# qic999/PCTrans

Measured on AMD Instinct MI355X. Metric: MSDeformAttn+decoder fwd samples/sec at 512x512, 100 queries, higher is better.
Workload: dtype bf16 decoder (autocast) / f32 MSDeformAttn pixel decoder

## Files before the change

include/pctrans_hip.h:

```cpp
#ifndef PCTRANS_HIP_H_
#define PCTRANS_HIP_H_

#include <stdint.h>

#ifdef __cplusplus
extern "C" {
#endif

#define PCT_ABI_VERSION 1

#define PCT_API __attribute__((visibility("default")))

#define PCT_OK 0
#define PCT_ERR_BAD_ARG (-1)
#define PCT_ERR_IM2COL_STEP (-2)
#define PCT_ERR_ALIGNMENT (-3)
#define PCT_ERR_UNSUPPORTED (-4)

PCT_API int pct_abi_version(void);
PCT_API const char *pct_error_string(int code);
PCT_API const char *pct_build_info(void);
PCT_API int pct_prepare_device(void);

PCT_API int pct_ms_deform_attn_forward_f32(const float *value, const int64_t *spatial_shapes, const int64_t *level_start,
// ... 7 lines not shown
PCT_API int pct_ms_deform_attn_forward_f16(const void *value, const int64_t *spatial_shapes, const int64_t *level_start,
                                   const float *sampling_loc, const float *attn_weight, int batch,
                                   int spatial_size, int num_heads, int channels, int num_levels, int num_query,
                                   int num_point, int im2col_step, void *output, void *stream);
PCT_API int pct_ms_deform_attn_forward_bf16(const void *value, const int64_t *spatial_shapes, const int64_t *level_start,
                                    const float *sampling_loc, const float *attn_weight, int batch,
                                    int spatial_size, int num_heads, int channels, int num_levels, int num_query,
                                    int num_point, int im2col_step, void *output, void *stream);

PCT_API int pct_ms_deform_attn_fused_forward_f32(const float *value, const int64_t *spatial_shapes,
                                                 const int64_t *level_start, const float *ref_points,
                                                 long long ref_batch_stride, const float *offsets,
                                                 const float *attn_logits, int batch, int spatial_size, int num_heads,
                                                 int channels, int num_levels, int num_query, int num_point,
                                                 float *output, void *stream);

PCT_API int pct_ms_deform_attn_forward_planes_f32(const float *value_planes, const int64_t *spatial_shapes,
                                                  const int64_t *level_start, const float *loc_planes,
                                                  const float *attn_planes, const float *ref_points,
                                                  long long ref_batch_stride, int batch, int spatial_size, int num_heads,
                                                  int channels, int num_levels, int num_query, int num_point,
                                                  float *output, void *stream);

PCT_API int pct_ms_deform_attn_backward_f32(const float *value, const int64_t *spatial_shapes, const int64_t *level_start,
                                    const float *sampling_loc, const float *attn_weight, const float *grad_output,
                                    int batch, int spatial_size, int num_heads, int channels, int num_levels,
                                    int num_query, int num_point, int im2col_step, float *grad_value,
                                    float *grad_sampling_loc, float *grad_attn_weight, void *stream);
PCT_API int pct_ms_deform_attn_backward_f64(const double *value, const int64_t *spatial_shapes, const int64_t *level_start,
                                    const double *sampling_loc, const double *attn_weight,
                                    const double *grad_output, int batch, int spatial_size, int num_heads,
                                    int channels, int num_levels, int num_query, int num_point, int im2col_step,
                                    double *grad_value, double *grad_sampling_loc, double *grad_attn_weight,
                                    void *stream);

PCT_API int pct_dynamic_mask_head_forward(const float *mask_feat, const float *ref_points, const float *params,
                                          int batch, int channels, int num_query, int height, int width, int stride,
                                          int rel_coord, int target_h, int target_w, int out_dtype, void *up_logits,
                                          unsigned char *attn_mask, void *stream);

PCT_API int pct_dynamic_mask_head_forward_mfma(const float *mask_feat, const float *ref_points, const float *params,
                                               int batch, int channels, int num_query, int height, int width,
                                               int stride, int rel_coord, int target_h, int target_w, void *scratch,
                                               void *up_logits, unsigned char *attn_mask, void *stream);

PCT_API int pct_dynamic_mask_head_forward_fused_bf16(const float *mask_feat, const float *ref_points, const float *params,
                                                     int batch, int channels, int num_query, int height, int width,
                                                     int stride, int rel_coord, int target_h, int target_w,
                                                     void *workspace, void *up_logits, unsigned char *attn_mask,
                                                     void *stream);

#include "pctrans_hip_train.h"
#include "pctrans_hip_post.h"

PCT_API int pct_add_layernorm_f32(const float *x, const float *y, const float *gamma, const float *beta, float eps,
                                  long long rows, int cols, float *out, void *stream);

PCT_API int pct_groupnorm_flatten_f32(const float *x, const float *gamma, const float *beta, int batch, int channels,
                                      int hw, int groups, float eps, float *stats, float *out,
                                      long long out_batch_stride, long long out_offset, void *stream);

PCT_API int pct_linear_k128_f32(const float *x, long long ldx, const float *x_add, long long ld_add, long long add_period,
                                const float *w, const float *bias, long long rows, int n, int act, float *y,
                                long long ldy, void *stream);
PCT_API void pct_msda_set_kernel_choice(int choice);
PCT_API int pct_msda_last_kernel(void);
PCT_API void pct_msda_set_bwd_kernel_choice(int choice);
PCT_API int pct_msda_last_bwd_kernel(void);

PCT_API int pct_linear_k128_multi_f32(const float *x, long long ldx, const float *x_add, long long ld_add,
                                      long long add_period, int nseg, const float *const *w, const float *const *bias,
                                      const int *n, const int *use_add, float *const *y, const long long *ldy,
                                      long long rows, void *stream);
PCT_API int pct_linear_k128_add_layernorm_f32(const float *x, long long ldx, const float *w, const float *bias,
                                              const float *residual, long long ldr, const float *gamma,
                                              const float *beta, float eps, long long rows, float *out,
                                              long long ldo, void *stream);

PCT_API int pct_linear_add_layernorm_f32(const float *x, long long ldx, int k, const float *w, void *w_split_ws,
                                         const float *bias, const float *residual, long long ldr, const float *gamma,
                                         const float *beta, float eps, long long rows, float *out, long long ldo,
                                         void *stream);

PCT_API int pct_ffn_layernorm_f32(const float *x, long long ldx, const float *w1, const float *b1, const float *w2,
                                  const float *b2, const float *gamma, const float *beta, float eps, int hidden,
                                  long long rows, void *w_image_ws, float *out, long long ldo, void *stream);

PCT_API int pct_conv1x1_groupnorm_tokens_f32(const float *x, const float *w, const float *bias, void *w_split_ws,
                                             const float *gamma, const float *beta, int groups, float eps, int batch,
                                             int in_channels, int out_channels, int hw, float *partial_ws, float *stats,
                                             float *out, long long out_batch_stride, long long out_offset, void *stream);

PCT_API int pct_conv1x1_nchw_f32(const float *x, const float *w, const float *bias, void *w_split_ws, int batch,
                                 int in_channels, int out_channels, int hw, float *out, void *stream);

PCT_API int pct_lsap_f32(const float *cost, int batch, int num_query, int ld_target, const int *num_target,
                         int *row_for_target, int *status, void *stream);

PCT_API int pct_masked_attention_bf16(const void *q, const void *k, const void *vT, const unsigned char *mask,
                                      int batch, int heads, int num_query, int num_key, int head_dim,
                                      int v_head_dim, float scale, int out_dtype, void *out, void *stream);

PCT_API int pct_cross_attention_bf16(const void *q_content, const void *q_pos, const void *k_content, const void *k_pos,
                                     const void *v, const unsigned char *mask, const unsigned char *row_open, int batch,
                                     int heads, int num_query, int num_key, float scale, void *out, void *stream);

// ... 5 lines not shown
```

pctrans_amd/_lib.py:

```python
import ctypes
import os

_HERE = os.path.dirname(os.path.abspath(__file__))
LIB_PATH = os.path.join(_HERE, "lib", "libpctrans_hip.so")
ABI_VERSION = 1

_lib = None

_vp, _i = ctypes.c_void_p, ctypes.c_int
_FWD_ARGS = [_vp, _vp, _vp, _vp, _vp, _i, _i, _i, _i, _i, _i, _i, _i, _vp, _vp]
_BWD_ARGS = [_vp, _vp, _vp, _vp, _vp, _vp, _i, _i, _i, _i, _i, _i, _i, _i, _vp, _vp, _vp, _vp]

SYMBOLS = {
    "pct_abi_version": ([], _i),
    "pct_error_string": ([_i], ctypes.c_char_p),
    "pct_build_info": ([], ctypes.c_char_p),
    "pct_prepare_device": ([], _i),
    "pct_ms_deform_attn_forward_f32": (_FWD_ARGS, _i),
    "pct_ms_deform_attn_forward_f64": (_FWD_ARGS, _i),
    "pct_ms_deform_attn_forward_f16": (_FWD_ARGS, _i),
    "pct_ms_deform_attn_forward_bf16": (_FWD_ARGS, _i),
    "pct_ms_deform_attn_backward_f32": (_BWD_ARGS, _i),
    "pct_ms_deform_attn_backward_f64": (_BWD_ARGS, _i),
    "pct_ms_deform_attn_fused_forward_f32": ([_vp, _vp, _vp, _vp, ctypes.c_longlong, _vp, _vp] + [_i] * 7 + [_vp, _vp], _i),
# ... 4 lines not shown
    "pct_msda_set_kernel_choice": ([_i], None),
    "pct_msda_last_kernel": ([], _i),
    "pct_msda_set_bwd_kernel_choice": ([_i], None),
    "pct_msda_last_bwd_kernel": ([], _i),
    "pct_linear_k128_multi_f32": ([_vp, ctypes.c_longlong, _vp, ctypes.c_longlong, ctypes.c_longlong, _i, _vp, _vp, _vp, _vp,
                                   _vp, _vp, ctypes.c_longlong, _vp], _i),
    "pct_linear_k128_add_layernorm_f32": ([_vp, ctypes.c_longlong, _vp, _vp, _vp, ctypes.c_longlong, _vp, _vp,
                                           ctypes.c_float, ctypes.c_longlong, _vp, ctypes.c_longlong, _vp], _i),
    "pct_linear_add_layernorm_f32": ([_vp, ctypes.c_longlong, _i, _vp, _vp, _vp, _vp, ctypes.c_longlong, _vp, _vp,
                                      ctypes.c_float, ctypes.c_longlong, _vp, ctypes.c_longlong, _vp], _i),
    "pct_groupnorm_flatten_f32": ([_vp, _vp, _vp, _i, _i, _i, _i, ctypes.c_float, _vp, _vp, ctypes.c_longlong,
                                   ctypes.c_longlong, _vp], _i),
    "pct_conv1x1_nchw_f32": ([_vp, _vp, _vp, _vp, _i, _i, _i, _i, _vp, _vp], _i),
    "pct_conv1x1_groupnorm_tokens_f32": ([_vp] * 6 + [_i, ctypes.c_float] + [_i] * 4 + [_vp, _vp, _vp, ctypes.c_longlong,
                                          ctypes.c_longlong, _vp], _i),
    "pct_ffn_layernorm_f32": ([_vp, ctypes.c_longlong, _vp, _vp, _vp, _vp, _vp, _vp, ctypes.c_float, _i, ctypes.c_longlong, _vp, _vp,
                               ctypes.c_longlong, _vp], _i),
    "pct_lsap_f32": ([_vp, _i, _i, _i, _vp, _vp, _vp, _vp], _i),
    "pct_cross_attention_bf16": ([_vp] * 7 + [_i] * 4 + [ctypes.c_float, _vp, _vp], _i),
    "pct_masked_attention_bf16": ([_vp, _vp, _vp, _vp] + [_i] * 6 + [ctypes.c_float, _i, _vp, _vp], _i),
    "pct_dynamic_mask_head_forward_mfma": ([_vp, _vp, _vp] + [_i] * 9 + [_vp, _vp, _vp, _vp], _i),
    "pct_dynamic_mask_head_forward_fused_bf16": ([_vp, _vp, _vp] + [_i] * 9 + [_vp, _vp, _vp, _vp], _i),
    "pct_dynamic_mask_head_forward": ([_vp, _vp, _vp] + [_i] * 10 + [_vp, _vp, _vp], _i),
}

OPT_IN_SYMBOLS = {
    "pct_dynamic_mask_head_backward_f32": ([_vp, _vp, _vp, _vp] + [_i] * 7 + [_vp, _vp, _vp, _vp, _vp], _i,
                                           "tests/test_dmh_train_gpu.py"),
    "pct_point_sample_f32": ([_vp, _vp, _vp] + [_i] * 7 + [_vp, _vp], _i, "tests/test_point_loss_gpu.py"),
    "pct_point_mask_loss_forward_f32": ([_vp, _vp, _i, _i, _i, _vp, _vp, _i, _i, _i, _vp, _i, _i, _vp, _vp, _vp, _vp], _i,
                                        "tests/test_point_loss_gpu.py"),
    "pct_point_mask_loss_backward_f32": ([_vp] * 6 + [_i] * 4 + [_vp, _vp], _i, "tests/test_point_loss_gpu.py"),
    "pct_point_select_uncertain_f32": ([_vp, _vp, _i, _i, _i, _vp, _i, _i, _i, _vp, _i, _vp, _vp], _i,
                                       "tests/test_point_select_gpu.py"),
    "pct_point_match_cost_f32": ([_vp, _i, _i, _i, _i, _vp, _i, _i, _i, _vp, _vp, _i, _vp, _i, ctypes.c_float, ctypes.c_float,
                                  _vp, _vp, _vp], _i, "tests/test_match_cost_gpu.py"),
    "pct_instance_label_map_f32": ([_vp, _i, _i, _i, _vp, _vp, _i, _i, _i, _vp, _vp], _i, "tests/test_embedding_loss_gpu.py"),
    "pct_discriminative_loss_forward_f32": ([_vp, _vp] + [_i] * 5 + [ctypes.c_float] * 5 + [_vp] * 5, _i,
                                            "tests/test_embedding_loss_gpu.py"),
    "pct_discriminative_loss_backward_f32": ([_vp] * 4 + [_i] * 5 + [ctypes.c_float, _vp, _vp], _i,
                                             "tests/test_embedding_loss_gpu.py"),
}

_POST_MASKS = [_vp] + [_i] * 7 + [_vp, _vp, _vp]
_POST_LABELS = [_vp] + [_i] * 7 + [_vp, _vp, _vp]
POST_SYMBOLS = {
    "pct_instance_masks_f32": (_POST_MASKS, _i, "tests/test_postprocess_gpu.py"),
    "pct_instance_masks_bf16": (_POST_MASKS, _i, "tests/test_postprocess_gpu.py"),
    "pct_instance_labels_from_bits": ([_vp, _vp] + [_i] * 5 + [_vp, _vp, _vp], _i, "tests/test_postprocess_gpu.py"),
    "pct_instance_labels_f32": (_POST_LABELS, _i, "tests/test_postprocess_gpu.py"),
    "pct_instance_labels_bf16": (_POST_LABELS, _i, "tests/test_postprocess_gpu.py"),
}


class PctransLibraryError(RuntimeError):
    pass


def lib():
    global _lib
    if _lib is not None:
        return _lib
    if not os.path.exists(LIB_PATH):
        raise PctransLibraryError(
            "libpctrans_hip.so not found at %s -- build it with `make -C pctrans_amd/csrc` "
            "(or `python -c 'import __graft_entry__ as g; g.build()'`).  "
            "pctrans_amd has no CPU / eager fallback for device tensors." % LIB_PATH)
    l = ctypes.CDLL(LIB_PATH)
    for name, (argtypes, restype) in list(SYMBOLS.items()) + [
            (k, v[:2]) for k, v in list(OPT_IN_SYMBOLS.items()) + list(POST_SYMBOLS.items())]:
        try:
            fn = getattr(l, name)
        except AttributeError as e:
            raise PctransLibraryError("libpctrans_hip.so does not export %s (stale build?)" % name) from e
        fn.argtypes = argtypes
        fn.restype = restype
    v = l.pct_abi_version()
    if v != ABI_VERSION:
        raise PctransLibraryError("libpctrans_hip.so ABI version %d, expected %d -- rebuild" % (v, ABI_VERSION))
    _lib = l
    return _lib


def check(code, what):
    if code != 0:
        msg = lib().pct_error_string(code).decode()
        raise RuntimeError("%s failed: %s (code %d)" % (what, msg, code))


_PREPARED = set()


def prepare_device(device):
    import torch
    idx = device.index if device.index is not None else torch.cuda.current_device()
    if idx in _PREPARED:
        return
    if torch.cuda.is_current_stream_capturing():
        return
    with torch.cuda.device(idx):
        check(lib().pct_prepare_device(), "prepare_device")
    _PREPARED.add(idx)
```

pctrans_amd/csrc/c_abi.hip:

```cpp
#include <hip/hip_runtime.h>
#include <stdint.h>

#include "launchers.hpp"
#include "msda_common.hpp"

namespace {

int check_common(const void *value, const int64_t *shapes, const int64_t *starts, const void *loc,
                 const void *attn, int N, int S, int M, int D, int L, int Lq, int P, int im2col_step,
                 size_t elem, size_t loc_elem)
{
  if (N < 0 || S < 0 || Lq < 0 || M <= 0 || D <= 0 || L <= 0 || P <= 0 || im2col_step <= 0) return PCT_ERR_BAD_ARG;
  if (N == 0) return PCT_OK;
  const int step = N < im2col_step ? N : im2col_step;
  if (N % step != 0) return PCT_ERR_IM2COL_STEP;
  if (Lq == 0) return PCT_OK;
  if (!value || !shapes || !starts || !loc || !attn) return PCT_ERR_BAD_ARG;
  if ((long long)S * M * D >= 0x7fffffffLL) return PCT_ERR_UNSUPPORTED;
  if ((uintptr_t)value % elem || (uintptr_t)loc % loc_elem || (uintptr_t)attn % loc_elem ||
      (uintptr_t)shapes % 8 || (uintptr_t)starts % 8)
    return PCT_ERR_ALIGNMENT;
  return PCT_OK;
}

// ... 96 lines not shown
}

int instance_labels_impl(const void *logits, int bf16, int batch, int num_query, int h, int w, int height, int width, int dataset,
                         void *workspace, int16_t *labels, void *stream)
{
  const int rc = check_instance_post(batch, num_query, h, w, height, width, dataset);
  if (rc != PCT_OK || batch == 0) return rc;
  if (num_query == 0) return instance_labels_empty(batch, height, width, labels, stream);
  if (!logits || !workspace || !labels) return PCT_ERR_BAD_ARG;
  if (((uintptr_t)logits & (bf16 ? 1u : 3u)) || ((uintptr_t)workspace & 15u) || ((uintptr_t)labels & 1u)) return PCT_ERR_ALIGNMENT;
  return pct::launch_instance_labels(logits, bf16, batch, num_query, h, w, height, width, dataset, workspace, labels,
                                     static_cast<hipStream_t>(stream));
}

}

extern "C" {

int pct_instance_masks_f32(const float *logits, int batch, int num_query, int h, int w, int height, int width, int dataset,
                           uint32_t *bits, int32_t *areas, void *stream)
{
  return instance_masks_impl(logits, 0, batch, num_query, h, w, height, width, dataset, bits, areas, stream);
}

int pct_instance_masks_bf16(const void *logits, int batch, int num_query, int h, int w, int height, int width, int dataset,
                            uint32_t *bits, int32_t *areas, void *stream)
{
  return instance_masks_impl(logits, 1, batch, num_query, h, w, height, width, dataset, bits, areas, stream);
}

int pct_instance_labels_from_bits(const uint32_t *bits, const int32_t *areas, int batch, int num_query, int height, int width,
                                  int dataset, void *workspace, int16_t *labels, void *stream)
{
  const int rc = check_instance_post(batch, num_query, 1, 1, height, width, dataset);
  if (rc != PCT_OK || batch == 0) return rc;
  if (num_query == 0) return instance_labels_empty(batch, height, width, labels, stream);
  if (!bits || !areas || !workspace || !labels) return PCT_ERR_BAD_ARG;
  if (((uintptr_t)bits & 15u) || ((uintptr_t)areas & 3u) || ((uintptr_t)workspace & 15u) || ((uintptr_t)labels & 1u))
    return PCT_ERR_ALIGNMENT;
  return pct::launch_instance_labels_from_bits(bits, areas, batch, num_query, height, width, dataset, workspace, labels,
                                               static_cast<hipStream_t>(stream));
}

int pct_instance_labels_f32(const float *logits, int batch, int num_query, int h, int w, int height, int width, int dataset,
                            void *workspace, int16_t *labels, void *stream)
{
  return instance_labels_impl(logits, 0, batch, num_query, h, w, height, width, dataset, workspace, labels, stream);
}

int pct_instance_labels_bf16(const void *logits, int batch, int num_query, int h, int w, int height, int width, int dataset,
                             void *workspace, int16_t *labels, void *stream)
{
  return instance_labels_impl(logits, 1, batch, num_query, h, w, height, width, dataset, workspace, labels, stream);
}

int pct_abi_version(void) { return PCT_ABI_VERSION; }

const char *pct_error_string(int code)
{
  switch (code) {
    case PCT_OK: return "ok";
    case PCT_ERR_BAD_ARG: return "bad argument (null pointer or non-positive size)";
    case PCT_ERR_IM2COL_STEP: return "batch must be divisible by min(batch, im2col_step)";
    case PCT_ERR_ALIGNMENT: return "pointer not aligned to its element size";
    case PCT_ERR_UNSUPPORTED: return "shape not supported by the gfx950 kernels";
    default: break;
  }
  if (code > 0) return hipGetErrorString(static_cast<hipError_t>(code));
  return "unknown error";
}

int pct_ms_deform_attn_forward_f32(const float *value, const int64_t *spatial_shapes, const int64_t *level_start,
                                   const float *sampling_loc, const float *attn_weight, int batch,
                                   int spatial_size, int num_heads, int channels, int num_levels, int num_query,
                                   int num_point, int im2col_step, float *output, void *stream)
{
  return forward_impl<float, float>(value, spatial_shapes, level_start, sampling_loc, attn_weight, batch,
                                    spatial_size, num_heads, channels, num_levels, num_query, num_point,
                                    im2col_step, output, stream);
}

int pct_ms_deform_attn_forward_f64(const double *value, const int64_t *spatial_shapes, const int64_t *level_start,
                                   const double *sampling_loc, const double *attn_weight, int batch,
                                   int spatial_size, int num_heads, int channels, int num_levels, int num_query,
                                   int num_point, int im2col_step, double *output, void *stream)
{
  return forward_impl<double, double>(value, spatial_shapes, level_start, sampling_loc, attn_weight, batch,
                                      spatial_size, num_heads, channels, num_levels, num_query, num_point,
                                      im2col_step, output, stream);
}

int pct_ms_deform_attn_forward_f16(const void *value, const int64_t *spatial_shapes, const int64_t *level_start,
                                   const float *sampling_loc, const float *attn_weight, int batch,
                                   int spatial_size, int num_heads, int channels, int num_levels, int num_query,
                                   int num_point, int im2col_step, void *output, void *stream)
{
  return forward_impl<pct::half_bits, float>(value, spatial_shapes, level_start, sampling_loc, attn_weight, batch,
                                             spatial_size, num_heads, channels, num_levels, num_query, num_point,
                                             im2col_step, output, stream);
}

int pct_ms_deform_attn_forward_bf16(const void *value, const int64_t *spatial_shapes, const int64_t *level_start,
                                    const float *sampling_loc, const float *attn_weight, int batch,
                                    int spatial_size, int num_heads, int channels, int num_levels, int num_query,
                                    int num_point, int im2col_step, void *output, void *stream)
{
// ... 435 lines not shown
```

pctrans_amd/csrc/launchers.hpp:

```cpp
#pragma once
#include <hip/hip_runtime.h>
#include <stdint.h>

#include "../../include/pctrans_hip.h"

namespace pct {

constexpr int PCT_NOT_COVERED = -100;

enum MsdaFwdKernel { MSDA_FWD_AUTO = 0, MSDA_FWD_WIN = 1, MSDA_FWD_GENERIC = 2, MSDA_FWD_QUAD = 3, MSDA_FWD_COL = 4 };
enum MsdaBwdKernel { MSDA_BWD_AUTO = 0, MSDA_BWD_WIN = 1, MSDA_BWD_GENERIC = 2, MSDA_BWD_COL = 3 };

template <typename T>
int launch_msda_forward(const void *value, const int64_t *shapes, const int64_t *starts, const void *loc, const void *attn, int N,
                        int S, int M, int D, int L, int Lq, int P, void *out, hipStream_t stream);
template <typename T>
int launch_msda_forward_special(const void *value, const int64_t *shapes, const int64_t *starts, const void *loc,
                                const void *attn, int N, int S, int M, int D, int L, int Lq, int P, void *out, hipStream_t stream,
                                const float *ref, long long ref_batch_stride);
int launch_msda_forward_planes(const void *value, const int64_t *shapes, const int64_t *starts, const void *loc, const void *attn,
                               int N, int S, int M, int D, int L, int Lq, int P, void *out, hipStream_t stream, const float *ref,
                               long long ref_batch_stride);
template <typename T>
int launch_msda_forward_win(const void *value, const int64_t *shapes, const int64_t *starts, const void *loc, const void *attn,
// ... 22 lines not shown
int launch_msda_backward_win(const float *value, const int64_t *shapes, const int64_t *starts, const float *loc,
                             const float *attn, const float *grad_out, int N, int S, int M, int D, int L, int Lq, int P,
                             float *grad_value, float *grad_loc, float *grad_attn, hipStream_t stream);
int launch_msda_backward_col(const float *value, const int64_t *shapes, const int64_t *starts, const float *loc,
                             const float *attn, const float *grad_out, int N, int S, int M, int D, int L, int Lq, int P,
                             float *grad_value, float *grad_loc, float *grad_attn, bool forced, hipStream_t stream);
void set_msda_bwd_kernel_choice(int c);
int msda_bwd_kernel_choice();
void note_msda_bwd_kernel(int k);
int msda_bwd_last_kernel();

unsigned *win_queue_slot(hipStream_t stream);
int prepare_win_queue_device();
int prepare_msda_backward_col_device();
int prepare_ffn_device();

int launch_dyn_mask_head(const float *feat, const float *ref, const float *params, int N, int C, int Q, int H, int W, int stride,
                         int rel_coord, int th, int tw, int out_dtype, void *up, unsigned char *amask, hipStream_t stream);
int launch_dyn_mask_head_mfma(const float *feat, const float *ref, const float *params, int N, int C, int Q, int H, int W,
                              int stride, int rel_coord, int th, int tw, void *scratch, void *up, unsigned char *amask,
                              hipStream_t stream);
int launch_dyn_mask_head_fused(const float *feat, const float *ref, const float *params, int N, int C, int Q, int H, int W,
                               int stride, int rel_coord, int th, int tw, void *workspace, void *up, unsigned char *amask,
                               hipStream_t stream);
int launch_dyn_mask_head_bwd(const float *feat, const float *ref, const float *params, const float *grad_up, int N, int C, int Q,
                             int H, int W, int stride, int rel_coord, void *workspace, float *grad_feat, float *grad_ref,
                             float *grad_params, hipStream_t stream);

int launch_linear_k128(const float *x, long long ldx, const float *x2, long long ldx2, long long x2_period, const float *w,
                       const float *bias, long long rows, int n, int epi, float *y, long long ldy, const float *residual,
                       long long ldr, const float *gamma, const float *beta, float eps, hipStream_t stream);
int launch_linear_k128_split(const float *x, long long ldx, const float *x2, long long ldx2, long long x2_period, const float *w,
                             const float *bias, long long rows, int n, int epi, float *y, long long ldy, const float *residual,
                             long long ldr, const float *gamma, const float *beta, float eps, hipStream_t stream);
int launch_linear_k128_split_multi(const float *x, long long ldx, const float *x2, long long ldx2, long long x2_period, int nseg,
                                   const float *const *w, const float *const *bias, const int *n, const int *use_add,
                                   float *const *y, const long long *ldy, long long rows, hipStream_t stream);
int launch_linear_ln_split(const float *x, long long ldx, const float *w, unsigned short *w_pieces, int K, const float *bias,
                           const float *residual, long long ldr, const float *gamma, const float *beta, float eps, long long rows,
                           float *out, long long ldo, hipStream_t stream);
int launch_ffn_fused_split(const float *x, long long ldx, const float *w1, const float *b1, const float *w2, const float *b2,
                           const float *gamma, const float *beta, float eps, int F, long long rows, void *img_ws, float *out,
                           long long ldo, hipStream_t stream);
int launch_conv1x1_nchw_split(const float *x, const float *w, const float *bias, unsigned short *w_split_ws, int N, int K, int HW,
                              float *y, hipStream_t stream);
int launch_conv1x1_groupnorm_tokens(const float *x, const float *w, const float *bias, unsigned short *w_split_ws,
                                    const float *gamma, const float *beta, float eps, int N, int K, int HW, float *partial_ws,
                                    float *stats, float *out, long long out_batch_stride, hipStream_t stream);
int launch_add_layernorm(const float *x, const float *y, const float *gamma, const float *beta, float eps, long long rows,
                         int cols, float *out, hipStream_t stream);
int launch_groupnorm_flatten(const float *x, const float *gamma, const float *beta, int N, int C, int HW, int groups, float eps,
                             float *stats, float *out, long long out_batch_stride, long long out_offset, hipStream_t stream);

int launch_masked_attention(const void *q, const void *k, const void *vT, const unsigned char *mask, int N, int heads, int Q,
                            int S, int head_dim, int v_head_dim, float scale, int out_dtype, void *out, hipStream_t stream);
int launch_cross_attention(const void *q_c, const void *q_s, const void *k_c, const void *k_p, const void *v,
                           const unsigned char *mask, const unsigned char *row_open, int N, int heads, int Q, int S, float scale,
                           void *out, hipStream_t stream);
int launch_lsap(const float *cost, int batch, int num_query, int ld_target, const int *num_target, int *row_for_target,
                int *status, hipStream_t stream);

int launch_point_sample(const float *planes, const int *plane_index, const float *coords, int num_planes, int H, int W, int K,
                        int P, int per_row, float *out, hipStream_t stream);
int launch_point_loss_forward(const float *pred, const int *src_index, int num_pred, int H, int W, const float *tgt,
                              const int *tgt_index, int num_tgt, int Ht, int Wt, const float *coords, int K, int P, float *x,
                              float *t, float *sums, hipStream_t stream);
int launch_point_loss_backward(const float *x, const float *t, const float *coords, const float *alpha, const float *beta,
                               const float *gamma, int K, int P, int H, int W, float *grad_planes, hipStream_t stream);
int launch_point_select(const float *pred, const int *src_index, int num_pred, int H, int W, const float *cand_coords, int K, int S,
                        int num_keep, float *out_coords, int out_row_points, int *out_index, hipStream_t stream);
int launch_point_match_cost(const float *pred, int B, int Q, int H, int W, const float *tgt, int num_tgt, int Ht, int Wt,
                            const int *tgt_start, const int *tgt_count, int Gmax, const float *coords, int P, float cost_mask,
                            float cost_dice, void *workspace, float *cost, hipStream_t stream);

int launch_instance_label_map(const float *planes, int num_planes, int Ht, int Wt, const int *start, const int *count, int B, int h,
                              int w, int *labels, hipStream_t stream);
int launch_emb_loss_forward(const float *emb, const int *labels, int B, int E, int h, int w, int L, float delta_v, float delta_d,
                            float alpha, float beta, float gama, void *workspace, float *table, float *loss, int *status,
                            hipStream_t stream);
int launch_emb_loss_backward(const float *emb, const int *labels, const float *table, const float *grad_out, int B, int E, int h,
                             int w, int L, float delta_v, float *grad_emb, hipStream_t stream);

int instance_geometry_status(int N, int Q, int H, int W);
int launch_instance_masks(const void *logits, int bf16, int N, int Q, int h, int w, int H, int W, int dataset, unsigned *bits,
                          int *areas, hipStream_t stream);
int launch_instance_labels_from_bits(const unsigned *bits, const int *areas, int N, int Q, int H, int W, int dataset,
                                     void *workspace, short *labels, hipStream_t stream);
int launch_instance_labels(const void *logits, int bf16, int N, int Q, int h, int w, int H, int W, int dataset, void *workspace,
                           short *labels, hipStream_t stream);

}
```

pctrans_amd/fused_ops.py:

```python
import contextlib

import torch
from torch.nn import functional as F

from . import _lib, _timing


def _fusable(*tensors):
    if torch.is_grad_enabled() and any(t is not None and t.requires_grad for t in tensors):
        return False
    return all(t is None or (t.is_cuda and t.dtype == torch.float32) for t in tensors)


def add_layer_norm(x, y, norm):
    cols = x.shape[-1]
    if (not _fusable(x, y, norm.weight, norm.bias) or cols not in (64, 128, 256) or norm.weight is None
            or norm.bias is None or tuple(norm.normalized_shape) != (cols,) or (y is not None and y.shape != x.shape)):
        return norm(x if y is None else x + y)
    xc = x.contiguous()
    yc = y.contiguous() if y is not None else None
    out = torch.empty_like(xc)
    rows = xc.numel() // cols
    with torch.cuda.device(x.device):
        rc = _lib.lib().pct_add_layernorm_f32(
# ... 235 lines not shown
            and w.dtype == torch.float32 and w.device == x.device and tuple(w.shape[2:]) == (1, 1) and w.shape[0] == 128
            and w.shape[1] == x.shape[1] and w.shape[1] % 16 == 0 and (x.shape[2] * x.shape[3]) % 128 == 0
            and tuple(conv.stride) == (1, 1) and tuple(conv.padding) == (0, 0) and tuple(conv.dilation) == (1, 1)
            and conv.groups == 1 and getattr(conv, "norm", None) is None and getattr(conv, "activation", None) is None
            and x.numel() > 0 and x.shape[0] * (x.shape[2] * x.shape[3] // 128) < 2 ** 31 - 1
            and x.data_ptr() % 16 == 0 and w.data_ptr() % 16 == 0 and w.is_contiguous()
            and (conv.bias is None or conv.bias.data_ptr() % 16 == 0) and not torch.is_autocast_enabled()
            and not (torch.is_grad_enabled() and (x.requires_grad or w.requires_grad)))


def conv1x1_nchw(x, conv):
    if not conv1x1_nchw_supported(x, conv):
        return conv(x)
    n, k, h, w_ = x.shape
    stream = torch.cuda.current_stream(x.device).cuda_stream
    key = (x.device, stream, k)
    ws = _CONV_WS.get(key)
    if ws is None:
        ws = _CONV_WS[key] = torch.empty((3, 128, k), dtype=torch.bfloat16, device=x.device)
    out = torch.empty((n, 128, h, w_), dtype=torch.float32, device=x.device)
    with torch.cuda.device(x.device), _timing.timed("conv1x1 k=%d" % k, x):
        rc = _lib.lib().pct_conv1x1_nchw_f32(
            x.data_ptr(), conv.weight.data_ptr(), conv.bias.data_ptr() if conv.bias is not None else None, ws.data_ptr(),
            n, k, 128, h * w_, out.data_ptr(), stream)
    _lib.check(rc, "conv1x1_nchw")
    return out


def conv1x1_groupnorm_tokens_supported(x, conv, gn):
    return (conv1x1_nchw_supported(x, conv) and isinstance(gn, torch.nn.GroupNorm) and gn.num_groups == 32
            and gn.num_channels == 128 and gn.weight is not None and gn.bias is not None
            and gn.weight.data_ptr() % 16 == 0 and gn.bias.data_ptr() % 16 == 0 and x.shape[0] <= 65535
            and not (torch.is_grad_enabled() and gn.weight.requires_grad))


def conv1x1_groupnorm_tokens_into(x, conv, gn, out, row_offset):
    n, k, h, w_ = x.shape
    hw = h * w_
    stream = torch.cuda.current_stream(x.device).cuda_stream
    key = (x.device, stream, k)
    ws = _CONV_WS.get(key)
    if ws is None:
        ws = _CONV_WS[key] = torch.empty((3, 128, k), dtype=torch.bfloat16, device=x.device)
    partial = torch.empty((n * (hw // 128) * 2 * 64,), dtype=torch.float32, device=x.device)
    stats = torch.empty((n * 64,), dtype=torch.float32, device=x.device)
    with torch.cuda.device(x.device), _timing.timed("conv1x1_gn k=%d" % k, x):
        rc = _lib.lib().pct_conv1x1_groupnorm_tokens_f32(
            x.data_ptr(), conv.weight.data_ptr(), conv.bias.data_ptr() if conv.bias is not None else None, ws.data_ptr(),
            gn.weight.data_ptr(), gn.bias.data_ptr(), 32, float(gn.eps), n, k, 128, hw, partial.data_ptr(), stats.data_ptr(),
            out.data_ptr(), out.stride(0), row_offset * 128, stream)
    _lib.check(rc, "conv1x1_groupnorm_tokens")


def groupnorm_flatten_supported(x, gn):
    return (x.is_cuda and x.dtype == torch.float32 and x.dim() == 4 and x.shape[1] == 128 and x.is_contiguous()
            and isinstance(gn, torch.nn.GroupNorm) and gn.num_channels == 128 and (128 // gn.num_groups) % 4 == 0
            and gn.weight is not None and gn.bias is not None and not torch.is_autocast_enabled()
            and not (torch.is_grad_enabled() and (x.requires_grad or gn.weight.requires_grad)))


def groupnorm_flatten_into(x, gn, out, row_offset):
    n, c, h, w = x.shape
    stats = torch.empty((n * gn.num_groups * 2,), dtype=torch.float32, device=x.device)
    with torch.cuda.device(x.device):
        rc = _lib.lib().pct_groupnorm_flatten_f32(
            x.data_ptr(), gn.weight.data_ptr(), gn.bias.data_ptr(), n, c, h * w, gn.num_groups, float(gn.eps),
            stats.data_ptr(), out.data_ptr(), out.stride(0), row_offset * c,
            torch.cuda.current_stream(x.device).cuda_stream)
    _lib.check(rc, "groupnorm_flatten")


def lsap_supported(cost):
    return cost.is_cuda and cost.dim() == 3 and cost.shape[1] <= 1024 and cost.shape[2] <= 512


def lsap(cost, num_target):
    c = cost.detach().float().contiguous()
    B, Q, Gm = c.shape
    nt = num_target.to(device=c.device, dtype=torch.int32).contiguous()
    rows = torch.empty((B, Gm), dtype=torch.int32, device=c.device)
    status = torch.empty((B,), dtype=torch.int32, device=c.device)
    with torch.cuda.device(c.device):
        rc = _lib.lib().pct_lsap_f32(c.data_ptr(), B, Q, Gm, nt.data_ptr(), rows.data_ptr(), status.data_ptr(),
                                     torch.cuda.current_stream(c.device).cuda_stream)
    _lib.check(rc, "lsap")
    return rows, status


def masked_attention_supported(q, k, v, num_heads, attn_mask, key_padding_mask, dropout_p, training, need_weights):
    if not (q.is_cuda and q.dtype == torch.bfloat16 and k.dtype == torch.bfloat16 and v.dtype == torch.bfloat16):
        return False
    if torch.is_grad_enabled() and (q.requires_grad or k.requires_grad or v.requires_grad):
        return False
    if need_weights or key_padding_mask is not None or (dropout_p > 0.0 and training):
        return False
    if q.shape[2] // num_heads not in (16, 32) or v.shape[2] // num_heads != 16:
        return False
    if attn_mask is not None:
        if attn_mask.dtype != torch.bool:
            return False
        L, N, S = q.shape[0], q.shape[1], k.shape[0]
        if tuple(attn_mask.shape) not in ((N, 1, L, S), (L, S)):
            return False
    return True


# ... 51 lines not shown
```

pctrans_amd/transformer_decoder/mask2former_transformer_decoder.py:

```python
import logging
import math
from typing import Optional

import torch
from torch import Tensor, nn
from torch.nn import functional as F

from .. import dynamic_mask_head as dmh
from .. import fused_ops
from ..layers import CachedLinear, Conv2d, c2_xavier_fill, get_norm
from .attention import MultiheadAttention
from .position_encoding import PositionEmbeddingSine


_SINE_TABLES = {}


_HEAD_TABLES = {}


def gen_sineembed_for_position(pos_tensor, temperature=20):
    key = (pos_tensor.device, temperature)
    tab = _SINE_TABLES.get(key)
    if tab is None:
# ... 282 lines not shown
        self.point_embed = MLP(hidden_dim, hidden_dim, 2 * points_num, 3)
        for m in (self.ref_point_head, self.query_scale, self.point_embed):
            _init_mlp(m)

        self.in_channels = mask_dim
        self.dynamic_mask_channels = 8
        self.controller_layers = 3
        self.dmh_train = dmh.train_default()
        self.mask_out_stride = 4
        self.rel_coord = rel_coord
        ch = self.dynamic_mask_channels
        first_in = self.in_channels + 2 if self.rel_coord else self.in_channels
        self.weight_nums = [first_in * ch] + [ch * ch] * (self.controller_layers - 2) + [ch]
        self.bias_nums = [ch] * (self.controller_layers - 1) + [1]
        self.num_gen_params = sum(self.weight_nums) + sum(self.bias_nums)
        self.controller = MLP(hidden_dim, hidden_dim, self.num_gen_params, 3)
        _init_mlp(self.controller)

        self.mask_head = Conv2d(hidden_dim, mask_dim, 1, padding=0)
        nn.init.kaiming_uniform_(self.mask_head.weight, a=1)
        nn.init.constant_(self.mask_head.bias, 0)

        self.sem_loss_on = sem_loss_on
        if self.sem_loss_on:
            conv_block = conv_with_kaiming_uniform(norm, activation=True)
            self.seg_head = nn.Sequential(conv_block(hidden_dim, hidden_dim, kernel_size=3, stride=1),
                                          conv_block(hidden_dim, hidden_dim, kernel_size=3, stride=1))
            self.logits = Conv2d(hidden_dim, 1, kernel_size=1, stride=1)
            prior_prob = 0.01
            nn.init.constant_(self.logits.bias, -math.log((1 - prior_prob) / prior_prob))

    @classmethod
    def from_config(cls, cfg, in_channels, mask_classification):
        mf = cfg.MODEL.MASK_FORMER
        assert mf.DEC_LAYERS >= 1
        return dict(in_channels=in_channels, mask_classification=mask_classification, hidden_dim=mf.HIDDEN_DIM,
                    num_queries=mf.NUM_OBJECT_QUERIES, nheads=mf.NHEADS, dim_feedforward=mf.DIM_FEEDFORWARD,
                    points_num=mf.POSITION_POINTS_NUM, dec_layers=mf.DEC_LAYERS - 1, pre_norm=mf.PRE_NORM,
                    enforce_input_project=mf.ENFORCE_INPUT_PROJ, mask_dim=cfg.MODEL.SEM_SEG_HEAD.MASK_DIM,
                    sem_loss_on=mf.SEMANTIC_LOSS_ON, norm=mf.SEMANTIC_NORM, rel_coord=mf.REL_COORD)

    def forward(self, x, targets, mask_features, mask=None, attn_mask_threshold=0.5, criterion=None):
        assert len(x) == self.num_feature_levels
        del mask
        graphed = self.__dict__.get("_pct_graphed_core")
        mf_lp = _lp(mask_features)
        if graphed is not None and self.training and torch.is_grad_enabled():
            flat = graphed(mask_features, *x)
        else:
            flat = self._forward_core(mask_features, *x, _mf_lp=mf_lp)
        n_pred = self.num_layers + 1
        output, outputs_coords = flat[0], flat[1]
        predictions_mask = list(flat[2:2 + n_pred])
        sem_logits_pred = self.logits(self.seg_head(mf_lp)) if self.sem_loss_on else None

        indices_list = []
        if targets is not None:
            many = getattr(criterion.matcher, "forward_many", None)
            if many is not None:
                indices_list = many([{"pred_masks": pm} for pm in predictions_mask], targets)
            else:
                indices_list = [criterion.matcher({"pred_masks": pm}, targets) for pm in predictions_mask]
            from .query_contrast import query_contrast_items
            contrast_items_query, contrast_items_mask = query_contrast_items(output, predictions_mask[-1], indices_list[-1])

        out = {
            "pred_masks": predictions_mask[-1],
            "aux_outputs": self._set_aux_loss(predictions_mask),
            "reference_points": outputs_coords[-1],
            "aux_reference_points": self._set_refpoints_aux_loss(outputs_coords),
            "indices_list": indices_list,
        }
        if targets is not None:
            out["pred_qd_query"] = contrast_items_query
            out["pred_qd_mask"] = contrast_items_mask
        if self.sem_loss_on:
            out["sem_mask"] = sem_logits_pred
        return out

    def _forward_core(self, mask_features, *x, _mf_lp=None):
        src, pos, size_list = [], [], []
        for i in range(self.num_feature_levels):
            size_list.append(x[i].shape[-2:])
            p = self.pe_layer(x[i], None).flatten(2)
            s = self.input_proj[i](x[i]).flatten(2) + self.level_embed.weight[i][None, :, None]
            pos.append(_lp(p.permute(2, 0, 1)))
            src.append(_lp(s.permute(2, 0, 1)))
        bs = src[0].shape[1]

        query_embed = _lp(self.query_embed.weight.unsqueeze(1).repeat(1, bs, 1))
        output = self.query_feat.weight.unsqueeze(1).repeat(1, bs, 1)

        predictions_mask, outputs_coords = [], []
        out_lp = None
        reference_points = self.ref_point_head(query_embed).sigmoid()
        ref_points = [reference_points]

        mf_lp = _mf_lp if _mf_lp is not None else _lp(mask_features)
        feats_f32 = None
        if fused_ops.conv1x1_from_token_rows_supported(mask_features, self.mask_head):
            mask_feat = feats_f32 = fused_ops.conv1x1_from_token_rows(mask_features, self.mask_head)
        else:
            mask_feat = self.mask_head(mf_lp)
        if feats_f32 is None and mask_feat.is_cuda and mask_feat.dtype != torch.float32 and not (
                torch.is_grad_enabled() and mask_feat.requires_grad):
            feats_f32 = mask_feat.float().contiguous()

# ... 123 lines not shown
```

Baseline: 1430.

## Fuse semantic seg head conv3x3+BN+ReLU chain and logits into MFMA kernels

```diff
diff --git a/include/pctrans_hip.h b/include/pctrans_hip.h
--- a/include/pctrans_hip.h
+++ b/include/pctrans_hip.h
@@ -83,6 +83,7 @@
 
 #include "pctrans_hip_train.h"
 #include "pctrans_hip_post.h"
+#include "pctrans_hip_seg.h"
 
 PCT_API int pct_add_layernorm_f32(const float *x, const float *y, const float *gamma, const float *beta, float eps,
                                   long long rows, int cols, float *out, void *stream);
diff --git a/include/pctrans_hip_seg.h b/include/pctrans_hip_seg.h
--- /dev/null
+++ b/include/pctrans_hip_seg.h
@@ -0,0 +1,22 @@
+#ifndef PCTRANS_HIP_SEG_H
+#define PCTRANS_HIP_SEG_H
+
+#ifdef __cplusplus
+extern "C" {
+#endif
+
+PCT_API int pct_conv3x3_bn_relu_bf16(const void *x, const float *w, const float *mean, const float *var, const float *gamma,
+                                     const float *beta, float eps, void *w_ws, int batch, int channels, int height, int width,
+                                     int channels_last, void *out, void *stream);
+
+PCT_API int pct_seg_head_bf16(const void *x, const float *w_a, const float *mean_a, const float *var_a, const float *gamma_a,
+                              const float *beta_a, float eps_a, const float *w_b, const float *mean_b, const float *var_b,
+                              const float *gamma_b, const float *beta_b, float eps_b, const float *w_logits,
+                              const float *b_logits, void *w_ws, void *mid, int batch, int channels, int height, int width,
+                              int channels_last, void *out, void *stream);
+
+#ifdef __cplusplus
+}
+#endif
+
+#endif
diff --git a/pctrans_amd/_lib.py b/pctrans_amd/_lib.py
--- a/pctrans_amd/_lib.py
+++ b/pctrans_amd/_lib.py
@@ -80,6 +80,12 @@
     "pct_instance_labels_bf16": (_POST_LABELS, _i, "tests/test_postprocess_gpu.py"),
 }
 
+SEG_SYMBOLS = {
+    "pct_conv3x3_bn_relu_bf16": ([_vp] * 6 + [ctypes.c_float, _vp] + [_i] * 5 + [_vp, _vp], _i, "tests/test_seg_head_gpu.py"),
+    "pct_seg_head_bf16": ([_vp] * 6 + [ctypes.c_float] + [_vp] * 5 + [ctypes.c_float] + [_vp] * 4 + [_i] * 5 + [_vp, _vp], _i,
+                          "tests/test_seg_head_gpu.py"),
+}
+
 
 class PctransLibraryError(RuntimeError):
     pass
@@ -96,7 +102,7 @@
             "pctrans_amd has no CPU / eager fallback for device tensors." % LIB_PATH)
     l = ctypes.CDLL(LIB_PATH)
     for name, (argtypes, restype) in list(SYMBOLS.items()) + [
-            (k, v[:2]) for k, v in list(OPT_IN_SYMBOLS.items()) + list(POST_SYMBOLS.items())]:
+            (k, v[:2]) for k, v in list(OPT_IN_SYMBOLS.items()) + list(POST_SYMBOLS.items()) + list(SEG_SYMBOLS.items())]:
         try:
             fn = getattr(l, name)
         except AttributeError as e:
diff --git a/pctrans_amd/csrc/c_abi.hip b/pctrans_amd/csrc/c_abi.hip
--- a/pctrans_amd/csrc/c_abi.hip
+++ b/pctrans_amd/csrc/c_abi.hip
@@ -172,6 +172,40 @@
                              void *workspace, int16_t *labels, void *stream)
 {
   return instance_labels_impl(logits, 1, batch, num_query, h, w, height, width, dataset, workspace, labels, stream);
+}
+
+int pct_conv3x3_bn_relu_bf16(const void *x, const float *w, const float *mean, const float *var, const float *gamma,
+                             const float *beta, float eps, void *w_ws, int batch, int channels, int height, int width,
+                             int channels_last, void *out, void *stream)
+{
+  if (batch < 0 || channels <= 0 || height <= 0 || width <= 0) return PCT_ERR_BAD_ARG;
+  if (batch == 0) return PCT_OK;
+  if (!x || !w || !mean || !var || !gamma || !beta || !w_ws || !out) return PCT_ERR_BAD_ARG;
+  if ((((uintptr_t)x | (uintptr_t)out) & (channels_last ? 15u : 1u)) ||
+      (((uintptr_t)w | (uintptr_t)mean | (uintptr_t)var | (uintptr_t)gamma | (uintptr_t)beta) & 3u) || ((uintptr_t)w_ws & 15u))
+    return PCT_ERR_ALIGNMENT;
+  const float *const bnp[4] = {mean, var, gamma, beta};
+  return abi_status(pct::launch_conv3x3_bn_relu(x, channels_last, w, bnp, eps, w_ws, batch, channels, height, width, out,
+                                                static_cast<hipStream_t>(stream)));
+}
+
+int pct_seg_head_bf16(const void *x, const float *w_a, const float *mean_a, const float *var_a, const float *gamma_a,
+                      const float *beta_a, float eps_a, const float *w_b, const float *mean_b, const float *var_b,
+                      const float *gamma_b, const float *beta_b, float eps_b, const float *w_logits, const float *b_logits, void *w_ws,
+                      void *mid, int batch, int channels, int height, int width, int channels_last, void *out, void *stream)
+{
+  if (batch < 0 || channels <= 0 || height <= 0 || width <= 0) return PCT_ERR_BAD_ARG;
+  if (batch == 0) return PCT_OK;
+  const float *const bn_a[4] = {mean_a, var_a, gamma_a, beta_a}, *const bn_b[4] = {mean_b, var_b, gamma_b, beta_b};
+  uintptr_t f32_bits = (uintptr_t)w_a | (uintptr_t)w_b | (uintptr_t)w_logits | (uintptr_t)b_logits;
+  for (int i = 0; i < 4; ++i) {
+    if (!bn_a[i] || !bn_b[i]) return PCT_ERR_BAD_ARG;
+    f32_bits |= (uintptr_t)bn_a[i] | (uintptr_t)bn_b[i];
+  }
+  if (!x || !w_a || !w_b || !w_logits || !w_ws || !mid || !out) return PCT_ERR_BAD_ARG;
+  if ((((uintptr_t)x | (uintptr_t)mid) & (channels_last ? 15u : 1u)) || ((uintptr_t)out & 1u) || (f32_bits & 3u) || ((uintptr_t)w_ws & 15u)) return PCT_ERR_ALIGNMENT;
+  return abi_status(pct::launch_seg_head(x, channels_last, w_a, bn_a, eps_a, w_b, bn_b, eps_b, w_logits, b_logits, w_ws, mid, batch, channels,
+                                         height, width, out, static_cast<hipStream_t>(stream)));
 }
 
 int pct_abi_version(void) { return PCT_ABI_VERSION; }
diff --git a/pctrans_amd/csrc/conv3x3_bn_relu.hip b/pctrans_amd/csrc/conv3x3_bn_relu.hip
--- /dev/null
+++ b/pctrans_amd/csrc/conv3x3_bn_relu.hip
@@ -0,0 +1,266 @@
+
+#include "launchers.hpp"
+#include "split_bf16.hpp"
+
+namespace pct {
+
+constexpr int S3_C = 128;
+constexpr int S3_TH = 8, S3_TW = 32;
+constexpr int S3_HW = S3_TW + 2;
+constexpr int S3_HP = (S3_TH + 2) * S3_HW;
+constexpr int S3_CS = 32;
+constexpr int S3_PS = 80;
+constexpr int S3_XBUF = S3_HP * S3_PS;
+constexpr int S3_WBUF = S3_C * S3_PS;
+constexpr int S3_BLOCK = 256;
+constexpr int S3_TASKS = S3_HP * (S3_CS / 8);
+constexpr int S3_ROUNDS = (S3_TASKS + S3_BLOCK - 1) / S3_BLOCK;
+constexpr int S3_STEP_ELEMS = S3_C * S3_CS;
+constexpr int S3_W_ELEMS = S3_C * S3_C * 9;
+
+__device__ __forceinline__ float s3_round_bf16(const float v) { return (float)(__bf16)v; }
+__device__ __forceinline__ unsigned short s3_bits_bf16(const float v) { return __builtin_bit_cast(unsigned short, (__bf16)v); }
+
+__global__ __launch_bounds__(256) void conv3x3_weight_image_kernel(const float *__restrict__ w0, const float *__restrict__ w1,
+                                                                   unsigned short *__restrict__ ws)
+{
+  const int e = blockIdx.x * 256 + threadIdx.x;
+  if (e >= S3_W_ELEMS) return;
+  const float *w = blockIdx.y ? w1 : w0;
+  const int ci_l = e & 31, co = (e >> 5) & 127, st = e >> 12, slab = st / 9, tap = st - slab * 9;
+  ws[(size_t)blockIdx.y * S3_W_ELEMS + e] = s3_bits_bf16(w[((size_t)co * S3_C + slab * S3_CS + ci_l) * 9 + tap]);
+}
+
+template <bool LOGITS, bool NHWC>
+__global__ __launch_bounds__(S3_BLOCK, 2) void conv3x3_bn_relu_kernel(
+    const unsigned short *__restrict__ x, const unsigned short *__restrict__ ws, const float *__restrict__ bn_mean,
+    const float *__restrict__ bn_var, const float *__restrict__ bn_gamma, const float *__restrict__ bn_beta, const float eps,
+    const float *__restrict__ w1, const float *__restrict__ b1, const int H, const int W, const int tiles_x, const int tiles_y,
+    unsigned short *__restrict__ y)
+{
+  __shared__ __attribute__((aligned(16))) unsigned char xs[S3_XBUF];
+  __shared__ __attribute__((aligned(16))) unsigned char wsm[2][S3_WBUF];
+  __shared__ f32x4 bn[S3_C];
+  __shared__ float w1s[S3_C];
+
+  const int tid = threadIdx.x, lane = tid & 63;
+  const int wave = __builtin_amdgcn_readfirstlane(tid >> 6);
+  const int tiles = tiles_x * tiles_y;
+  const int n = blockIdx.x / tiles, tile = blockIdx.x - n * tiles;
+  const int tyi = tile / tiles_x, y0 = tyi * S3_TH, x0 = (tile - tyi * tiles_x) * S3_TW;
+  const int HWp = H * W;
+  const unsigned short *xn = x + (size_t)n * S3_C * HWp;
+
+  if (tid < S3_C) {
+    bn[tid] = f32x4{bn_mean[tid], rsqrtf(bn_var[tid] + eps), bn_gamma[tid], bn_beta[tid]};
+    if constexpr (LOGITS) w1s[tid] = s3_round_bf16(w1[tid]);
+  }
+
+  int goff[S3_ROUNDS], loff[S3_ROUNDS];
+#pragma unroll
+  for (int rd = 0; rd < S3_ROUNDS; ++rd) {
+    const int task = rd * S3_BLOCK + tid;
+    const int cg = NHWC ? (task & 3) : task / S3_HP, p = NHWC ? (task >> 2) : task - cg * S3_HP;
+    const int py = p / S3_HW, px = p - py * S3_HW;
+    const int gy = y0 - 1 + py, gx = x0 - 1 + px;
+    const bool live = task < S3_TASKS;
+    const int pix = gy * W + gx;
+    goff[rd] = (live && gy >= 0 && gy < H && gx >= 0 && gx < W) ? (NHWC ? pix * S3_C + cg * 8 : cg * 8 * HWp + pix) : -1;
+    loff[rd] = live ? p * S3_PS + cg * 16 : -1;
+  }
+  unsigned short raw[8];
+  i32x4 gin[S3_ROUNDS], gw[2];
+  auto load_x = [&](const int slab, const int rd) {
+    if constexpr (NHWC) {
+      gin[rd] = goff[rd] >= 0 ? *reinterpret_cast<const i32x4 *>(xn + slab * S3_CS + goff[rd]) : i32x4{0, 0, 0, 0};
+    } else {
+      const unsigned short *p = xn + (size_t)slab * S3_CS * HWp + (goff[rd] >= 0 ? goff[rd] : 0);
+#pragma unroll
+      for (int j = 0; j < 8; ++j) raw[j] = goff[rd] >= 0 ? p[(size_t)j * HWp] : (unsigned short)0;
+    }
+  };
+  auto pack_x = [&](const int rd) {
+    if constexpr (!NHWC)
+      gin[rd] = i32x4{(int)(raw[0] | ((unsigned)raw[1] << 16)), (int)(raw[2] | ((unsigned)raw[3] << 16)),
+                      (int)(raw[4] | ((unsigned)raw[5] << 16)), (int)(raw[6] | ((unsigned)raw[7] << 16))};
+  };
+  auto stash_x = [&]() {
+#pragma unroll
+    for (int rd = 0; rd < S3_ROUNDS; ++rd)
+      if (loff[rd] >= 0) *reinterpret_cast<i32x4 *>(xs + loff[rd]) = gin[rd];
+  };
+  const int wl0 = (tid >> 2) * S3_PS + (tid & 3) * 16, wl1 = wl0 + 64 * S3_PS;
+  auto fetch_w = [&](const int step) {
+    const i32x4 *p = reinterpret_cast<const i32x4 *>(ws + (size_t)step * S3_STEP_ELEMS) + tid;
+    gw[0] = p[0];
+    gw[1] = p[S3_BLOCK];
+  };
+  auto stash_w = [&](const int buf) {
+    *reinterpret_cast<i32x4 *>(wsm[buf] + wl0) = gw[0];
+    *reinterpret_cast<i32x4 *>(wsm[buf] + wl1) = gw[1];
+  };
+
+  const int r = lane & 31, h = lane >> 5;
+  const int a_off = r * S3_PS + h * 16;
+  const int b_off = (2 * wave * S3_HW + r) * S3_PS + h * 16;
+
+  f32x16 acc[4][2];
+#pragma unroll
+  for (int rb = 0; rb < 4; ++rb)
+#pragma unroll
+    for (int cb = 0; cb < 2; ++cb)
+#pragma unroll
+      for (int j = 0; j < 16; ++j) acc[rb][cb][j] = 0.f;
+
+  fetch_w(0);
+#pragma unroll
+  for (int rd = 0; rd < S3_ROUNDS; ++rd) {
+    load_x(0, rd);
+    pack_x(rd);
+  }
+  stash_x();
+  stash_w(0);
+  __syncthreads();
+
+  for (int slab = 0; slab < S3_C / S3_CS; ++slab) {
+    const bool more_x = slab + 1 < S3_C / S3_CS;
+#pragma unroll
+    for (int tap = 0; tap < 9; ++tap) {
+      const int step = slab * 9 + tap, buf = step & 1;
+      const bool more_w = more_x || tap < 8;
+      if (more_w) fetch_w(step + 1);
+      if (tap < S3_ROUNDS && more_x) load_x(slab + 1, tap);
+      __builtin_amdgcn_sched_barrier(0);
+      const unsigned char *bp = xs + b_off + ((tap / 3) * S3_HW + tap % 3) * S3_PS;
+      const unsigned char *ap = wsm[buf] + a_off;
+#pragma unroll
+      for (int kk = 0; kk < 2; ++kk) {
+        bf16x8 wa[4], xb[2];
+#pragma unroll
+        for (int cb = 0; cb < 2; ++cb) xb[cb] = *reinterpret_cast<const bf16x8 *>(bp + cb * S3_HW * S3_PS + kk * 32);
+#pragma unroll
+        for (int rb = 0; rb < 4; ++rb) wa[rb] = *reinterpret_cast<const bf16x8 *>(ap + rb * 32 * S3_PS + kk * 32);
+#pragma unroll
+        for (int rb = 0; rb < 4; ++rb)
+#pragma unroll
+          for (int cb = 0; cb < 2; ++cb) acc[rb][cb] = mfma_bf16(wa[rb], xb[cb], acc[rb][cb]);
+      }
+      if (tap < S3_ROUNDS && more_x) pack_x(tap);
+      if (tap == 8 && more_x) {
+        __syncthreads();
+        stash_x();
+      }
+      if (more_w) stash_w(buf ^ 1);
+      __syncthreads();
+    }
+  }
+
+  const int gx = x0 + r;
+  if constexpr (LOGITS) {
+    const float bias = b1 ? b1[0] : 0.f;
+#pragma unroll
+    for (int cb = 0; cb < 2; ++cb) {
+      float s = 0.f;
+#pragma unroll
+      for (int rb = 0; rb < 4; ++rb)
+#pragma unroll
+        for (int q = 0; q < 4; ++q)
+#pragma unroll
+          for (int t = 0; t < 4; ++t) {
+            const int co = rb * 32 + 8 * q + 4 * h + t;
+            const f32x4 c = bn[co];
+            const float z = s3_round_bf16(acc[rb][cb][4 * q + t]);
+            const float a = fmaxf(s3_round_bf16(fmaf(c[2], (z - c[0]) * c[1], c[3])), 0.f);
+            s = fmaf(a, w1s[co], s);
+          }
+      s += __shfl_xor(s, 32);
+      const int gy = y0 + 2 * wave + cb;
+      if (h == 0 && gy < H && gx < W) y[((size_t)n * H + gy) * W + gx] = s3_bits_bf16(s + bias);
+    }
+    return;
+  }
+  unsigned short *yn = y + (size_t)n * S3_C * HWp;
+#pragma unroll
+  for (int rb = 0; rb < 4; ++rb)
+#pragma unroll
+    for (int q = 0; q < 4; ++q) {
+      const int co0 = rb * 32 + 8 * q + 4 * h;
+      f32x4 c[4];
+#pragma unroll
+      for (int t = 0; t < 4; ++t) c[t] = bn[co0 + t];
+#pragma unroll
+      for (int cb = 0; cb < 2; ++cb) {
+        const int gy = y0 + 2 * wave + cb;
+        const bool live = gy < H && gx < W;
+        const size_t pix = (size_t)gy * W + gx;
+        float a[4];
+#pragma unroll
+        for (int t = 0; t < 4; ++t) {
+          const float z = s3_round_bf16(acc[rb][cb][4 * q + t]);
+          a[t] = fmaxf(s3_round_bf16(fmaf(c[t][2], (z - c[t][0]) * c[t][1], c[t][3])), 0.f);
+        }
+        if constexpr (NHWC) {
+          const unsigned lo = s3_bits_bf16(a[0]) | ((unsigned)s3_bits_bf16(a[1]) << 16);
+          const unsigned hi = s3_bits_bf16(a[2]) | ((unsigned)s3_bits_bf16(a[3]) << 16);
+          if (live) *reinterpret_cast<uint2 *>(yn + pix * S3_C + co0) = uint2{lo, hi};
+        } else {
+#pragma unroll
+          for (int t = 0; t < 4; ++t)
+            if (live) yn[(size_t)(co0 + t) * HWp + pix] = s3_bits_bf16(a[t]);
+        }
+      }
+    }
+}
+
+namespace {
+
+bool s3_geometry_ok(int C, int H, int W, int &tiles_x, int &tiles_y)
+{
+  if (C != S3_C || H <= 0 || W <= 0 || (long long)H * W >= (1LL << 24)) return false;
+  tiles_x = (W + S3_TW - 1) / S3_TW;
+  tiles_y = (H + S3_TH - 1) / S3_TH;
+  return true;
+}
+
+template <bool LOGITS>
+void s3_launch(bool nhwc, long long grid, hipStream_t stream, const void *x, const unsigned short *ws, const float *const *bnp, float eps,
+               const float *w1, const float *b1, int H, int W, int tx, int ty, void *y)
+{
+  const auto kernel = nhwc ? conv3x3_bn_relu_kernel<LOGITS, true> : conv3x3_bn_relu_kernel<LOGITS, false>;
+  hipLaunchKernelGGL(kernel, dim3((unsigned)grid), dim3(S3_BLOCK), 0, stream, static_cast<const unsigned short *>(x), ws, bnp[0],
+                     bnp[1], bnp[2], bnp[3], eps, w1, b1, H, W, tx, ty, static_cast<unsigned short *>(y));
+}
+
+}
+
+int launch_conv3x3_bn_relu(const void *x, int nhwc, const float *w, const float *const *bnp, float eps, void *w_ws, int N, int C, int H,
+                           int W, void *out, hipStream_t stream)
+{
+  int tx, ty;
+  if (!s3_geometry_ok(C, H, W, tx, ty)) return PCT_NOT_COVERED;
+  if (N == 0) return 0;
+  const long long grid = (long long)N * tx * ty;
+  if (grid >= 0x7fffffffLL) return PCT_NOT_COVERED;
+  unsigned short *ws = static_cast<unsigned short *>(w_ws);
+  hipLaunchKernelGGL(conv3x3_weight_image_kernel, dim3((S3_W_ELEMS + 255) / 256, 1), dim3(256), 0, stream, w, w, ws);
+  s3_launch<false>(nhwc != 0, grid, stream, x, ws, bnp, eps, nullptr, nullptr, H, W, tx, ty, out);
+  return (int)hipGetLastError();
+}
+
+int launch_seg_head(const void *x, int nhwc, const float *w_a, const float *const *bn_a, float eps_a, const float *w_b,
+                    const float *const *bn_b, float eps_b, const float *w_logits, const float *b_logits, void *w_ws, void *mid,
+                    int N, int C, int H, int W, void *out, hipStream_t stream)
+{
+  int tx, ty;
+  if (!s3_geometry_ok(C, H, W, tx, ty)) return PCT_NOT_COVERED;
+  if (N == 0) return 0;
+  const long long grid = (long long)N * tx * ty;
+  if (grid >= 0x7fffffffLL) return PCT_NOT_COVERED;
+  unsigned short *ws = static_cast<unsigned short *>(w_ws);
+  hipLaunchKernelGGL(conv3x3_weight_image_kernel, dim3((S3_W_ELEMS + 255) / 256, 2), dim3(256), 0, stream, w_a, w_b, ws);
+  s3_launch<false>(nhwc != 0, grid, stream, x, ws, bn_a, eps_a, nullptr, nullptr, H, W, tx, ty, mid);
+  s3_launch<true>(nhwc != 0, grid, stream, mid, ws + S3_W_ELEMS, bn_b, eps_b, w_logits, b_logits, H, W, tx, ty, out);
+  return (int)hipGetLastError();
+}
+
+}
diff --git a/pctrans_amd/csrc/launchers.hpp b/pctrans_amd/csrc/launchers.hpp
--- a/pctrans_amd/csrc/launchers.hpp
+++ b/pctrans_amd/csrc/launchers.hpp
@@ -98,6 +98,12 @@
 int launch_groupnorm_flatten(const float *x, const float *gamma, const float *beta, int N, int C, int HW, int groups, float eps,
                              float *stats, float *out, long long out_batch_stride, long long out_offset, hipStream_t stream);
 
+int launch_conv3x3_bn_relu(const void *x, int nhwc, const float *w, const float *const *bnp, float eps, void *w_ws, int N, int C, int H,
+                           int W, void *out, hipStream_t stream);
+int launch_seg_head(const void *x, int nhwc, const float *w_a, const float *const *bn_a, float eps_a, const float *w_b,
+                    const float *const *bn_b, float eps_b, const float *w_logits, const float *b_logits, void *w_ws, void *mid,
+                    int N, int C, int H, int W, void *out, hipStream_t stream);
+
 int launch_masked_attention(const void *q, const void *k, const void *vT, const unsigned char *mask, int N, int heads, int Q,
                             int S, int head_dim, int v_head_dim, float scale, int out_dtype, void *out, hipStream_t stream);
 int launch_cross_attention(const void *q_c, const void *q_s, const void *k_c, const void *k_p, const void *v,
diff --git a/pctrans_amd/fused_ops.py b/pctrans_amd/fused_ops.py
--- a/pctrans_amd/fused_ops.py
+++ b/pctrans_amd/fused_ops.py
@@ -311,6 +311,97 @@
     _lib.check(rc, "conv1x1_groupnorm_tokens")
 
 
+_SEG_WS = {}
+
+
+def _seg_block_supported(x, block):
+    if not (isinstance(block, torch.nn.Sequential) and len(block) == 3):
+        return False
+    conv, bn, act = block[0], block[1], block[2]
+    if not (isinstance(conv, torch.nn.Conv2d) and isinstance(bn, torch.nn.modules.batchnorm._BatchNorm)
+            and isinstance(act, torch.nn.ReLU)):
+        return False
+    w = conv.weight
+    tensors = (w, bn.running_mean, bn.running_var, bn.weight, bn.bias)
+    return (tuple(w.shape) == (128, 128, 3, 3) and conv.bias is None and tuple(conv.stride) == (1, 1)
+            and tuple(conv.padding) == (1, 1) and tuple(conv.dilation) == (1, 1) and conv.groups == 1
+            and conv.padding_mode == "zeros" and getattr(conv, "norm", None) is None
+            and getattr(conv, "activation", None) is None and not bn.training and bn.num_features == 128
+            and all(t is not None and t.dtype == torch.float32 and t.device == x.device and t.is_contiguous()
+                    for t in tensors))
+
+
+def _seg_layout(x):
+    if x.is_contiguous():
+        return 0
+    n, c, h, w = x.shape
+    if x.stride() == (h * w * c, 1, w * c, c) and x.data_ptr() % 16 == 0:
+        return 1
+    return None
+
+
+def _seg_input_supported(x):
+    return (x.is_cuda and x.dtype == torch.bfloat16 and x.dim() == 4 and x.shape[1] == 128 and x.numel() > 0
+            and _seg_layout(x) is not None and x.shape[2] * x.shape[3] < 2 ** 24 and not torch.is_grad_enabled())
+
+
+def _seg_ws(x):
+    stream = torch.cuda.current_stream(x.device).cuda_stream
+    ws = _SEG_WS.get((x.device, stream))
+    if ws is None:
+        ws = _SEG_WS[(x.device, stream)] = torch.empty((2, 128 * 128 * 9), dtype=torch.bfloat16, device=x.device)
+    return ws, stream
+
+
+def _bn_args(bn):
+    return (bn.running_mean.data_ptr(), bn.running_var.data_ptr(), bn.weight.data_ptr(), bn.bias.data_ptr(), float(bn.eps))
+
+
+def conv3x3_bn_relu_supported(x, block):
+    return _seg_input_supported(x) and _seg_block_supported(x, block)
+
+
+def conv3x3_bn_relu(x, block):
+    if not conv3x3_bn_relu_supported(x, block):
+        return block(x)
+    n, _, h, w_ = x.shape
+    ws, stream = _seg_ws(x)
+    out = torch.empty_like(x)
+    with torch.cuda.device(x.device), _timing.timed("conv3x3_bn_relu", x):
+        rc = _lib.lib().pct_conv3x3_bn_relu_bf16(x.data_ptr(), block[0].weight.data_ptr(), *_bn_args(block[1]), ws.data_ptr(),
+                                                 n, 128, h, w_, _seg_layout(x), out.data_ptr(), stream)
+    _lib.check(rc, "conv3x3_bn_relu")
+    return out
+
+
+def seg_head_supported(x, seg_head, logits):
+    if not (_seg_input_supported(x) and isinstance(seg_head, torch.nn.Sequential) and len(seg_head) == 2
+            and all(_seg_block_supported(x, b) for b in seg_head) and isinstance(logits, torch.nn.Conv2d)):
+        return False
+    w, b = logits.weight, logits.bias
+    return (tuple(w.shape) == (1, 128, 1, 1) and tuple(logits.stride) == (1, 1) and tuple(logits.padding) == (0, 0)
+            and logits.groups == 1 and getattr(logits, "norm", None) is None and getattr(logits, "activation", None) is None
+            and w.dtype == torch.float32 and w.device == x.device and w.is_contiguous()
+            and (b is None or (b.dtype == torch.float32 and b.device == x.device)))
+
+
+def seg_head_forward(x, seg_head, logits):
+    if not seg_head_supported(x, seg_head, logits):
+        return logits(seg_head(x))
+    n, _, h, w_ = x.shape
+    ws, stream = _seg_ws(x)
+    mid = torch.empty_like(x)
+    out = torch.empty((n, 1, h, w_), dtype=torch.bfloat16, device=x.device)
+    a, b = seg_head[0], seg_head[1]
+    with torch.cuda.device(x.device), _timing.timed("seg_head", x):
+        rc = _lib.lib().pct_seg_head_bf16(
+            x.data_ptr(), a[0].weight.data_ptr(), *_bn_args(a[1]), b[0].weight.data_ptr(), *_bn_args(b[1]),
+            logits.weight.data_ptr(), logits.bias.data_ptr() if logits.bias is not None else None, ws.data_ptr(),
+            mid.data_ptr(), n, 128, h, w_, _seg_layout(x), out.data_ptr(), stream)
+    _lib.check(rc, "seg_head")
+    return out
+
+
 def groupnorm_flatten_supported(x, gn):
     return (x.is_cuda and x.dtype == torch.float32 and x.dim() == 4 and x.shape[1] == 128 and x.is_contiguous()
             and isinstance(gn, torch.nn.GroupNorm) and gn.num_channels == 128 and (128 // gn.num_groups) % 4 == 0
diff --git a/pctrans_amd/transformer_decoder/mask2former_transformer_decoder.py b/pctrans_amd/transformer_decoder/mask2former_transformer_decoder.py
--- a/pctrans_amd/transformer_decoder/mask2former_transformer_decoder.py
+++ b/pctrans_amd/transformer_decoder/mask2former_transformer_decoder.py
@@ -358,7 +358,7 @@
         n_pred = self.num_layers + 1
         output, outputs_coords = flat[0], flat[1]
         predictions_mask = list(flat[2:2 + n_pred])
-        sem_logits_pred = self.logits(self.seg_head(mf_lp)) if self.sem_loss_on else None
+        sem_logits_pred = fused_ops.seg_head_forward(mf_lp, self.seg_head, self.logits) if self.sem_loss_on else None
 
         indices_list = []
         if targets is not None:
```

Result: faster. 1465 (median of 6 runs) (+2.5%).
